# marcemq/crowdmod-ddpm-4D

Hardware: AMD Instinct MI355X
Metric: denoise-steps/sec (UNet fwd + sampler update) at ATC [B,4,T,H,W] (higher is better)
Workload: dtype f32; 1 GPU; config/ATC.yml sampling on the 12x36 grid, fp32 arithmetic (fp32 matrix instructions; fp32 products built from f16 two-way splits -- three v_mfma_f32_32x32x16_f16 cross terms, fp32 accumulate, same error against the reference as round 3's six-term bf16 form -- in the Winograd / quarter-resolution / last-conv layers, whose input is GroupNorm + SiLU output, and in the upsample layers, whose raw inpu; channels=4, past_len=5, future_len=3, global_batch=64, parallelism=batch-shard x1 (2 stream lanes of 32 chains per rank)

## Files before the change

### crowdmod-ddpm-4d_amd/csrc/cm_conv_wino.hip

```cpp
#include "cm_kernels.h"

#include <algorithm>
#include <atomic>
#include <map>
#include <mutex>
#include <tuple>
#include <vector>

namespace cm {

typedef float f32x16 __attribute__((ext_vector_type(16)));
typedef float f32x4 __attribute__((ext_vector_type(4)));
typedef _Float16 f16x8 __attribute__((ext_vector_type(8)));
typedef __bf16 bf16x8 __attribute__((ext_vector_type(8)));
typedef __bf16 bf16x4 __attribute__((ext_vector_type(4)));
typedef _Float16 f16x4 __attribute__((ext_vector_type(4)));

__device__ __forceinline__ float silu_w(float v) { return v * __builtin_amdgcn_rcpf(1.0f + __expf(-v)); }

typedef float f32x2 __attribute__((ext_vector_type(2)));
__device__ __forceinline__ f32x2 pk_sub2(f32x2 a, f32x2 b) {
  f32x2 r;
  asm("v_pk_add_f32 %0, %1, %2 neg_lo:[0,1] neg_hi:[0,1]" : "=v"(r) : "v"(a), "v"(b));
  return r;
// ... 390 lines not shown
  float *xb = XC + (size_t)(wave * 2) * 16 * 64 + lane;
#pragma unroll
  for (int reg = 0; reg < 16; ++reg) { xb[reg * 64] = t0[reg]; xb[(16 + reg) * 64] = t1[reg]; }
  __syncthreads();
  const int oa = wave >> 1, ob = wave & 1;
  f32x16 v;
  {
    const float *p0 = XC + (size_t)((0 * 2 + ob) * 16) * 64 + lane, *p1 = XC + (size_t)((1 * 2 + ob) * 16) * 64 + lane;
    const float *p2 = XC + (size_t)((2 * 2 + ob) * 16) * 64 + lane, *p3 = XC + (size_t)((3 * 2 + ob) * 16) * 64 + lane;
    if (oa == 0) {
#pragma unroll
      for (int reg = 0; reg < 16; ++reg) v[reg] = (p0[reg * 64] + p1[reg * 64]) + p2[reg * 64];
    } else {
#pragma unroll
      for (int reg = 0; reg < 16; ++reg) v[reg] = (p1[reg * 64] - p2[reg * 64]) - p3[reg * 64];
    }
  }
  if (n2 > 0) {
    for (int c0s = 0; c0s < n2; c0s += WINO_SKB) {
      if (c0s > 0) wino_skip_load(a, nt, n2a, n2, c0s, svox, lane, sa, sw);
      wino_skip_mfma(n2, c0s, sa, sw, v);
    }
  }
  wino_epilogue(a, v, outoff, nt, wave, lane, b0, bs, (((tz * a.nty + ty) * a.ntx) + tx) * 4 + wave, bias_pre, tv_pre);
}

#ifndef CM_WINO_ABL
#define CM_WINO_ABL 0
#endif
template <int BZ, int PY, int PX, bool F16, int NBW, bool SKIP, int B6 = 0, int FM = 0>
__global__ __launch_bounds__(256 * NBW, 2) void conv_wino_p_kernel(const ConvArgs a, const int *__restrict__ tabA,
                                                                  const int *__restrict__ tabO, int G) {
  constexpr bool ONE = (FM & WINO_FORM_ONE) != 0, PLAIN = (FM & WINO_FORM_PLAIN) != 0, OWNGN = (FM & WINO_FORM_OWNGN) != 0;
  constexpr bool WHOLE = (FM & WINO_FORM_WHOLE) != 0, AHEAD = (FM & WINO_FORM_AHEAD) != 0;
  static_assert(!AHEAD || (ONE && PLAIN && B6 == 3), "the halo-ahead order is a variant of the h2 one-sample forms");
  static_assert(!WHOLE || (BZ == 8 && PY == 2 && PX == 2 && NBW == 1), "the whole-tile form is the full-resolution tile's");
  static_assert(!OWNGN || PLAIN, "own GroupNorm is a variant of the plain activation form");
  constexpr int NT = 256 * NBW;
  constexpr int NP = PY * PX, ROWS = BZ * NP;
  static_assert(ROWS <= 32 && ROWS > 16, "one (partly filled) 32-row accumulator block per frequency component");
  constexpr int HZ = BZ + 2, UR = HZ * NP;
  static_assert(!(F16 && B6), "one operand format");
  constexpr bool SWZ = !F16 && !B6 && PY * PX == 4;
  constexpr bool CMP = B6 && BZ == 8;
  constexpr int URC = CMP ? (HZ - 1) * NP : UR;
  constexpr int CS = 16, S = CMP ? 24 : (B6 ? 28 : (F16 ? 12 : (SWZ ? CS : CS + 4)));
  constexpr int RYH = 2 * PY + 2, RXH = 2 * PX + 2, RV = HZ * RYH * RXH, RS_ = CMP ? 20 : (BZ == 8 ? 24 : 20);
  constexpr int PLV = RYH * RXH, RVC = CMP ? BZ * PLV : RV, RV0 = CMP ? PLV : 0;
  constexpr int RK = ((CMP ? BZ * RYH * RXH : RV) * 4 + NT - 1) / NT;
  constexpr int NITEMS = HZ * NP * (CS / 4);
  static_assert(NITEMS <= 256, "one staging item per thread");
  constexpr int USZ = 16 * URC * S, XSZ = NBW * 4 * 2 * 16 * 64;
  constexpr int UX = USZ > XSZ ? USZ : XSZ;
  extern __shared__ __attribute__((aligned(16))) float lds[];
  int *outoff = reinterpret_cast<int *>(lds);
  float *U = lds + 128;
  float *R = U + UX;
  float *GNL = R + RVC * RS_;

  const int tid = threadIdx.x, lane = tid & 63;
  const int wv8 = __builtin_amdgcn_readfirstlane(tid >> 6);
  const int wave = wv8 & 3, nbw = wv8 >> 2;
  const int r = lane & 31, hh = lane >> 5;
  const int g0 = blockIdx.x, p = blockIdx.y;
  const int nt = blockIdx.z * NBW + nbw;
  if (!ONE && g0 >= a.B) return;
  const int nc_epi = (WHOLE || nt * 32 + r < a.Co) ? nt * 32 + r : 0;
  const float bias_pre = a.bias[nc_epi];
// ... 91 lines not shown
      allv = allv && v4[0] >= 0 && v4[1] >= 0 && v4[2] >= 0 && v4[3] >= 0;
    }
  }
  const bool wave_all = WHOLE || (__all(allv) && nt * 32 + 31 < a.Co);
  const int n = nt * 32 + r;
  const bool nok = WHOLE || n < a.Co;
  const int n2a = SKIP ? a.s2C0 >> 5 : 0, n2 = SKIP ? (a.s2C0 + a.s2C1) >> 5 : 0;
  const int slot = p * 4 + wave;

  const bool own_gn = PLAIN ? OWNGN : a.gp0 != nullptr;
  const bool norm = PLAIN || a.gn != nullptr || own_gn;
  int b = g0;
  do {
    const bool more_b = !ONE && b + G < a.B;
    const float tv_pre = a.temb ? a.temb[(size_t)a.tidx[b] * a.temb_stride + nc_epi] : 0.f;
    if (own_gn) {
      __syncthreads();
      cm_gn_rows_from_slots(a, b, (int)Vs, GNL, U, tid, NT);
      __syncthreads();
    }
    f32x16 acc[4];
#pragma unroll
    for (int x = 0; x < 4; ++x)
#pragma unroll
      for (int i = 0; i < 16; ++i) acc[x][i] = 0.f;

    if constexpr (AHEAD) {
#pragma unroll
      for (int k = 0; k < RK; ++k) asm volatile("" : "+v"(ald[0][k]));
      if constexpr (!OWNGN) asm volatile("" : "+v"(scn[0]), "+v"(shn[0]));
      if (nchunks > 1) issue(NSL - 1, b, 1);
      asm volatile("" ::: "memory");
    }
    const int npair = AHEAD ? (nchunks & ~1) : nchunks;
#pragma unroll
    for (int pass = 0; pass < NSL; ++pass)
    for (int ch0 = pass ? npair : 0; ch0 < (pass ? nchunks : npair); ch0 += NSL)
#pragma unroll
    for (int SL = 0; SL < NSL - pass; ++SL) {
      const int ch = ch0 + SL;
      f32x4 sc1 = scn[SL], sh1 = shn[SL];
      if (own_gn) {
        const int cb0 = (ch < n0 ? ch * CS : a.C0 + (ch - n0) * CS) + 4 * aq;
        sc1 = *reinterpret_cast<const f32x4 *>(GNL + cb0);
        sh1 = *reinterpret_cast<const f32x4 *>(GNL + Ctot + cb0);
      }
      f32x4 pm1 = {1.f, 1.f, 1.f, 1.f};
      if (!((CM_WINO_ABL & 32) && ch > 0)) {
      if constexpr (!PLAIN) {
        if (a.pm) pm1 = *reinterpret_cast<const f32x4 *>(a.pm + (size_t)b * a.pm_stride + (ch < n0 ? ch * CS : a.C0 + (ch - n0) * CS) + 4 * aq);
      }
      if (PLAIN || (norm && a.silu && !a.pm)) {
#pragma unroll
        for (int k = 0; k < RK; ++k) {
          const int v = (tid >> 2) + (NT / 4) * k + RV0;
          f32x4 w = ald[SL][k] * sc1 + sh1;
          w[0] = silu_w(w[0]); w[1] = silu_w(w[1]); w[2] = silu_w(w[2]); w[3] = silu_w(w[3]);
          if (!((aok >> k) & 1u)) w = f32x4{0.f, 0.f, 0.f, 0.f};
          if (v >= RV0 && v < RV0 + RVC) *reinterpret_cast<f32x4 *>(R + (v - RV0) * RS_ + 4 * aq) = w;
        }
      } else {
#pragma unroll
        for (int k = 0; k < RK; ++k) {
          const int v = (tid >> 2) + (NT / 4) * k + RV0;
          f32x4 w = ald[SL][k];
          if (norm) {
            w = w * sc1 + sh1;
            if (a.silu) { w[0] = silu_w(w[0]); w[1] = silu_w(w[1]); w[2] = silu_w(w[2]); w[3] = silu_w(w[3]); }
          }
          if (a.pm) w = w * pm1;
          if (!((aok >> k) & 1u)) w = f32x4{0.f, 0.f, 0.f, 0.f};
          if (v >= RV0 && v < RV0 + RVC) *reinterpret_cast<f32x4 *>(R + (v - RV0) * RS_ + 4 * aq) = w;
        }
      }
      }
      __syncthreads();
      if constexpr (CMP) {
        if (ch == 0)
          for (int i = tid; i < 16 * 2 * NP * 3; i += NT) {
            const int xi = i / (2 * NP * 3), rem = i - xi * (2 * NP * 3), hf2 = rem / (NP * 3), r4 = rem - hf2 * (NP * 3);
            *reinterpret_cast<f32x4 *>(U + (size_t)xi * URC * S + (size_t)hf2 * URC * 12 + 4 * r4) = f32x4{0.f, 0.f, 0.f, 0.f};
          }
      }
      if (stager && !((CM_WINO_ABL & 4) && ch > 0)) {
        f32x4 d[16];
#pragma unroll
        for (int i = 0; i < 4; ++i)
#pragma unroll
          for (int j = 0; j < 4; ++j) d[i * 4 + j] = *reinterpret_cast<const f32x4 *>(R + rbase + (i * RXH + j) * RS_);
        auto put = [&](int k, const f32x4 v) {
          if constexpr (B6) {
            constexpr int NTW = B6 >= 2 ? 2 : 3;
            cm_u32x2_t t3[3];
            if constexpr (B6 == 3) cm_split2_f16(v, t3);
            else cm_split3_bf16<NTW>(v, t3);
#pragma unroll
            for (int tm = 0; tm < NTW; ++tm) *reinterpret_cast<cm_u32x2_t *>(uw + (size_t)k * URC * S + TST * tm) = t3[tm];
          } else if constexpr (F16) {
            const f16x4 hv = {(_Float16)v[0], (_Float16)v[1], (_Float16)v[2], (_Float16)v[3]};
            *reinterpret_cast<f16x4 *>(uw + (size_t)k * URC * S) = hv;
          } else {
            *reinterpret_cast<f32x4 *>(uw + (size_t)k * URC * S) = v;
          }
        };
        if constexpr (HX2) {
          f32x4 c[4][2];
// ... 11 lines not shown
            put(0 * 4 + j, pk_sub(e0, e2)); put(1 * 4 + j, e1 + e2); put(2 * 4 + j, pk_sub(e2, e1)); put(3 * 4 + j, pk_sub(e1, e3));
          }
        } else {
#pragma unroll
          for (int i = 0; i < 4; ++i) {
            const f32x4 e0 = d[i * 4 + 0], e1 = d[i * 4 + 1], e2 = d[i * 4 + 2], e3 = d[i * 4 + 3];
            d[i * 4 + 0] = pk_sub(e0, e2); d[i * 4 + 1] = e1 + e2; d[i * 4 + 2] = pk_sub(e2, e1); d[i * 4 + 3] = pk_sub(e1, e3);
          }
#pragma unroll
          for (int j = 0; j < 4; ++j) {
            const f32x4 e0 = d[0 * 4 + j], e1 = d[1 * 4 + j], e2 = d[2 * 4 + j], e3 = d[3 * 4 + j];
            d[0 * 4 + j] = pk_sub(e0, e2); d[1 * 4 + j] = e1 + e2; d[2 * 4 + j] = pk_sub(e2, e1); d[3 * 4 + j] = pk_sub(e1, e3);
          }
#pragma unroll
          for (int k = 0; k < 16; ++k) put(k, d[k]);
        }
      }
      __syncthreads();
#if !(CM_WINO_ABL & 2)
      if constexpr (!AHEAD) {
        if (ch + 1 < nchunks) issue(0, b, ch + 1);
        else if (more_b) issue(0, b + G, 0);
      }
#endif
      auto aread = [&](int g, f32x4 (&af)[4]) {
        const int dz = F16 ? g : g >> 1, k8 = F16 ? 0 : g & 1;
        const int acol = SWZ ? 4 * ((2 * k8 + hh) ^ (((ar >> 2) + dz) & 3)) : 8 * k8;
#pragma unroll
        for (int x = 0; x < 4; ++x) af[x] = *reinterpret_cast<const f32x4 *>(arow + (size_t)x * URC * S + (size_t)dz * NP * S + acol);
      };
      if constexpr (B6) {
        const float *ab = arow;
        f32x4 af6[2][3];
#pragma unroll
        for (int tm = 0; tm < 3; ++tm) af6[0][tm] = *reinterpret_cast<const f32x4 *>(ab + rowoff[0] + TST * tm);
#pragma unroll
        for (int sx = 0; sx < 12; ++sx) {
          const int g = sx >> 2, x = sx & 3;
          (void)g; (void)x;
          if (sx + 1 < 12) {
            const int g1 = (sx + 1) >> 2, x1 = (sx + 1) & 3;
#pragma unroll
            for (int tm = 0; tm < 3; ++tm)
              af6[(sx + 1) & 1][tm] = *reinterpret_cast<const f32x4 *>(ab + (size_t)x1 * URC * S + rowoff[g1] + TST * tm);
          }
          constexpr int TA[6] = {0, 2, 1, 0, 1, 0}, TB[6] = {2, 0, 1, 1, 0, 0};
#pragma unroll
          for (int u = (B6 >= 2 ? 3 : 0); u < ((CM_WINO_ABL & 8) ? (B6 >= 2 ? 4 : 1) : 6); ++u) {
            if constexpr (B6 == 3)
              acc[x] = __builtin_amdgcn_mfma_f32_32x32x16_f16(__builtin_bit_cast(f16x8, af6[sx & 1][TA[u]]),
                                                              __builtin_bit_cast(f16x8, b6[sx % RD6][TB[u]]), acc[x], 0, 0, 0);
            else
              acc[x] = __builtin_amdgcn_mfma_f32_32x32x16_bf16(__builtin_bit_cast(bf16x8, af6[sx & 1][TA[u]]),
                                                               __builtin_bit_cast(bf16x8, b6[sx % RD6][TB[u]]), acc[x], 0, 0, 0);
          }
          {
            constexpr int CHS = 4 * NG * 4 * 3 * 64;
            const int sn = sx + RD6;
            const bool wraps = sn >= 12;
            const bool more = !wraps || ch + 1 < nchunks || more_b;
            const int cn = !wraps ? ch : (ch + 1 < nchunks ? ch + 1 : 0);
            const f32x4 *wn = wbase + (size_t)cn * CHS + (size_t)((wraps ? sn - 12 : sn) * 3) * 64;
#if !(CM_WINO_ABL & 1)
            if (more) {
#pragma unroll
              for (int tm = 0; tm < 3; ++tm) b6[sx % RD6][tm] = wn[tm * 64];
            }
#else
            (void)wn; (void)more;
#endif
          }
          asm volatile("" ::: "memory");
        }
#if !(CM_WINO_ABL & 2)
        if constexpr (AHEAD) {
          if (pass == 0 && ch + 2 < nchunks) issue(SL, b, ch + 2);
          asm volatile("" ::: "memory");
        }
#endif
      } else {
#pragma unroll
      for (int g = 0; g < NG; ++g) {
        {
          const bool more = g < NG - 1 || ch + 1 < nchunks || more_b;
          const int cn = g < NG - 1 ? ch : (ch + 1 < nchunks ? ch + 1 : 0);
          const f32x4 *wn = wbase + (size_t)cn * (4 * NG * 4 * 64) + (size_t)(g < NG - 1 ? g + 1 : 0) * (4 * 64);
          if (more) {
#pragma unroll
            for (int x = 0; x < 4; ++x) bq[(g + 1) % RS][x] = wn[x * 64];
          }
        }
        f32x4 af[4];
        aread(g, af);
        if constexpr (F16) {
#pragma unroll
          for (int x = 0; x < 4; ++x)
            acc[x] = __builtin_amdgcn_mfma_f32_32x32x16_f16(__builtin_bit_cast(f16x8, af[x]), __builtin_bit_cast(f16x8, bq[g % RS][x]), acc[x], 0, 0, 0);
        } else {
#pragma unroll
          for (int jj = 0; jj < 4; ++jj)
#pragma unroll
            for (int x = 0; x < 4; ++x)
              acc[x] = __builtin_amdgcn_mfma_f32_32x32x2f32(af[x][jj], bq[g % RS][x][jj], acc[x], 0, 0, 0);
// ... 337 lines not shown
bool conv_wino_b6_ok(int bz, int by, int bx, int Co, int Zo) {
  if (cm::diag_env("CM_NO_WINO_P") || !conv_wino_tile_ok(bz, by, bx)) return false;
  const int nbw = conv_wino_nbw(bz, Co);
  if (bz != 8) return nbw == 2 && conv_wino_p_lds(bz, by, bx, false, 2, true) <= 160 * 1024;
  return nbw == 1 && by == 4 && bx == 4 && Zo == 8 && 2 * conv_wino_p_lds(bz, by, bx, false, 1, true) <= 160 * 1024 && !cm::diag_env("CM_NO_WINO_B6_FULL");
}

static size_t wino_p_lds_launch(const ConvArgs &a, bool f16, int nbw, bool b6, bool own_gn) {
  return conv_wino_p_lds(a.bz, a.by, a.bx, f16, nbw, b6) + (own_gn ? (size_t)2 * (a.C0 + a.C1) * sizeof(float) : 0);
}

bool conv_wino_p_taken(const ConvArgs &a, bool f16, bool own_gn) {
  static const bool no_p = cm::diag_env("CM_NO_WINO_P") != nullptr, all_p = cm::diag_env("CM_WINO_P") != nullptr;
  const int nbw = conv_wino_nbw_run(a, f16);
  const bool b6 = a.f16 == 2 || a.f16 == 3 || a.f16 == 4;
  return !no_p && conv_wino_two_step(a.bz, a.by, a.bx, f16, nbw) && (nbw == 2 || all_p || b6) &&
         wino_p_lds_launch(a, f16, nbw, b6, own_gn) <= 160 * 1024;
}

int conv_wino_form(const ConvArgs &a, int G) {
  if (a.dbg != 0 || a.f16 != 4) return 0;
  if (G < a.B || a.pm || !a.silu) return 0;
  const bool own = a.gp0 != nullptr;
  if (own == (a.gn != nullptr)) return 0;
  if (a.bz == 8) {
    const bool whole = a.by == 4 && a.bx == 4 && a.Yo % 4 == 0 && a.Xo % 4 == 0 && a.Zo % 8 == 0 && a.Co % 32 == 0;
    if (own || !whole || conv_wino_nbw(a.bz, a.Co) != 1) return 0;
    return WINO_FORM_ONE | WINO_FORM_PLAIN | WINO_FORM_WHOLE;
  }
  if (conv_wino_nbw(a.bz, a.Co) != 2) return 0;
  return WINO_FORM_ONE | WINO_FORM_PLAIN | (own ? WINO_FORM_OWNGN : 0);
}

static std::atomic<long long> wino_form_launches[16], wino_ahead_launches;
void conv_wino_form_counts(long long counts[16], bool reset) {
  for (int i = 0; i < 16; ++i) counts[i] = reset ? wino_form_launches[i].exchange(0) : wino_form_launches[i].load();
}
long long conv_wino_ahead_count(bool reset) { return reset ? wino_ahead_launches.exchange(0) : wino_ahead_launches.load(); }

hipError_t launch_conv_wino(const ConvArgs &a_in, bool f16, hipStream_t st) {
  ConvArgs a = a_in;
  a.dbg = conv_dbg_flags();
  if (!conv_wino_ok(a)) return hipErrorInvalidValue;
  const int nbw = conv_wino_nbw_run(a, f16);
  const bool b6 = a.f16 == 2 || a.f16 == 3 || a.f16 == 4;
  const bool t3 = a.f16 == 3, h2 = a.f16 == 4;
  if (b6 && (f16 || !conv_wino_b6_ok(a.bz, a.by, a.bx, a.Co, a.Zo))) return hipErrorInvalidValue;
#define CM_WINO_ATTR(KERNEL)                                                                        \
    static bool attr_set[64] = {false};                                                             \
    int dev = 0;                                                                                    \
    (void)hipGetDevice(&dev);                                                                       \
    if (!attr_set[dev & 63]) {                                                                      \
      hipError_t e = hipFuncSetAttribute(reinterpret_cast<const void *>(KERNEL), hipFuncAttributeMaxDynamicSharedMemorySize, 160 * 1024); \
      if (e != hipSuccess) return e;                                                                \
      attr_set[dev & 63] = true;                                                                    \
    }
  if (conv_wino_p_taken(a, f16, a.gp0 != nullptr)) {
    const size_t ldsp = wino_p_lds_launch(a, f16, nbw, b6, a.gp0 != nullptr);
    const int ntp = a.ntz * a.nty * a.ntx, nz = (a.Co + 31) / 32 / nbw;
    const int per_cu = (nbw == 1 && 2 * ldsp <= 160 * 1024) ? 2 : 1;
    const int slots = wino_cu_count() * per_cu;
    static const int g_force = cm::diag_env("CM_WINO_G") ? atoi(cm::diag_env("CM_WINO_G")) : 0;
    const int G = g_force > 0 ? std::min(a.B, g_force) : (b6 && nbw == 1) ? a.B : std::max(1, std::min(a.B, slots / std::max(1, ntp * nz)));
    WinoTabs tb;
    hipError_t et = wino_tabs_get(a, 256 * nbw, &tb);
    if (et != hipSuccess) return et;
    const dim3 gridp((unsigned)G, (unsigned)ntp, (unsigned)nz);
    static const bool no_ahead = cm::diag_env("CM_NO_WINO_AHEAD") != nullptr;
    const int fm0 = nbw == conv_wino_nbw(a.bz, a.Co) ? conv_wino_form(a, G) : 0;
    const int fm = fm0 && !no_ahead ? fm0 | WINO_FORM_AHEAD : fm0;
    int fm_run = 0;
#define CM_WINO_PGO1(KERNEL, THREADS)                                                               \
  {                                                                                                 \
    CM_WINO_ATTR(KERNEL)                                                                            \
    wino_form_launches[fm_run & 15].fetch_add(1, std::memory_order_relaxed);                        \
    if (fm_run & WINO_FORM_AHEAD) wino_ahead_launches.fetch_add(1, std::memory_order_relaxed);      \
    hipLaunchKernelGGL(KERNEL, gridp, dim3(THREADS), ldsp, st, a, tb.tA, tb.tO, G);                 \
    return hipGetLastError();                                                                       \
  }
#define CM_WINO_PGO(Z, PY_, PX_, F, NB, THREADS)                                                    \
  {                                                                                                 \
    if (a.s2w) CM_WINO_PGO1((conv_wino_p_kernel<Z, PY_, PX_, F, NB, true>), THREADS)                \
    CM_WINO_PGO1((conv_wino_p_kernel<Z, PY_, PX_, F, NB, false>), THREADS)                          \
  }
#define CM_WINO_PGOFM(Z, PY_, PX_, NB, THREADS, FM_)                                                \
    if (h2 && fm == (FM_)) {                                                                        \
      fm_run = (FM_);                                                                               \
      if (a.s2w) CM_WINO_PGO1((conv_wino_p_kernel<Z, PY_, PX_, false, NB, true, 3, (FM_)>), THREADS) \
      CM_WINO_PGO1((conv_wino_p_kernel<Z, PY_, PX_, false, NB, false, 3, (FM_)>), THREADS)          \
    }
#define CM_WINO_PGO6N(Z, PY_, PX_, NB, THREADS)                                                     \
  {                                                                                                 \
    if (h2) {                                                                                       \
      if (a.s2w) CM_WINO_PGO1((conv_wino_p_kernel<Z, PY_, PX_, false, NB, true, 3>), THREADS)       \
      CM_WINO_PGO1((conv_wino_p_kernel<Z, PY_, PX_, false, NB, false, 3>), THREADS)                 \
    }                                                                                               \
    if (t3) {                                                                                       \
      if (a.s2w) CM_WINO_PGO1((conv_wino_p_kernel<Z, PY_, PX_, false, NB, true, 2>), THREADS)       \
      CM_WINO_PGO1((conv_wino_p_kernel<Z, PY_, PX_, false, NB, false, 2>), THREADS)                 \
    }                                                                                               \
    if (a.s2w) CM_WINO_PGO1((conv_wino_p_kernel<Z, PY_, PX_, false, NB, true, 1>), THREADS)         \
    CM_WINO_PGO1((conv_wino_p_kernel<Z, PY_, PX_, false, NB, false, 1>), THREADS)                   \
  }
#define CM_WINO_PGO61(Z, PY_, PX_, THREADS) CM_WINO_PGO6N(Z, PY_, PX_, 1, THREADS)
#define CM_WINO_PGO6(Z, PY_, PX_, THREADS) CM_WINO_PGO6N(Z, PY_, PX_, 2, THREADS)
#define X(z, py, px)                                                                                \
    if (a.bz == z && a.by == 2 * py && a.bx == 2 * px) {                                            \
      if constexpr (z != 8) {                                                                       \
        if (nbw == 2 && b6) {                                                                       \
          CM_WINO_PGOFM(z, py, px, 2, 512, WINO_FORM_ONE | WINO_FORM_PLAIN)                         \
          CM_WINO_PGOFM(z, py, px, 2, 512, WINO_FORM_ONE | WINO_FORM_PLAIN | WINO_FORM_OWNGN)       \
          CM_WINO_PGOFM(z, py, px, 2, 512, WINO_FORM_ONE | WINO_FORM_PLAIN | WINO_FORM_AHEAD)       \
          CM_WINO_PGOFM(z, py, px, 2, 512, WINO_FORM_ONE | WINO_FORM_PLAIN | WINO_FORM_OWNGN | WINO_FORM_AHEAD) \
          CM_WINO_PGO6(z, py, px, 512)                                                              \
        }                                                                                           \
        if (nbw == 2 && f16) CM_WINO_PGO(z, py, px, true, 2, 512)                                   \
        if (nbw == 2) CM_WINO_PGO(z, py, px, false, 2, 512)                                         \
      }                                                                                             \
      if (f16) CM_WINO_PGO(z, py, px, true, 1, 256)                                                 \
      if constexpr (z == 8 && py == 2 && px == 2) {                                                 \
        if (b6) {                                                                                   \
          CM_WINO_PGOFM(z, py, px, 1, 256, WINO_FORM_ONE | WINO_FORM_PLAIN | WINO_FORM_WHOLE)       \
          CM_WINO_PGOFM(z, py, px, 1, 256, WINO_FORM_ONE | WINO_FORM_PLAIN | WINO_FORM_WHOLE | WINO_FORM_AHEAD) \
          CM_WINO_PGO61(z, py, px, 256)                                                             \
        }                                                                                           \
        CM_WINO_PGO(z, py, px, false, 1, 256)                                                       \
      }                                                                                             \
    }
    CM_WINO_TILES(X)
#undef X
  }
  if (b6) return hipErrorInvalidValue;
  if (a.gp0) return hipErrorInvalidValue;
  const dim3 grid((unsigned)(a.B * a.ntz * a.nty * a.ntx), (unsigned)((a.Co + 31) / 32 / nbw));
  const size_t lds = conv_wino_lds(a.bz, a.by, a.bx, f16, nbw);
#define CM_WINO_GO(KERNEL, THREADS)                                                                 \
  {                                                                                                 \
    CM_WINO_ATTR(KERNEL)                                                                            \
    hipLaunchKernelGGL(KERNEL, grid, dim3(THREADS), lds, st, a);                                    \
    return hipGetLastError();                                                                       \
  }
#define X(z, py, px)                                                                                \
  if (a.bz == z && a.by == 2 * py && a.bx == 2 * px) {                                              \
    constexpr bool two = (z == 8 && py == 2 && px == 2);                                            \
    if constexpr (z != 8) {                                                                         \
      if (nbw == 2 && f16) CM_WINO_GO((conv_wino_kernel<z, py, px, 2, true, true, 2>), 512)         \
      if (nbw == 2) CM_WINO_GO((conv_wino_kernel<z, py, px, 2, false, true, 2>), 512)               \
    }                                                                                               \
    if (f16) CM_WINO_GO((conv_wino_kernel<z, py, px, 2, true, true, 1>), 256)                       \
    CM_WINO_GO((conv_wino_kernel<z, py, px, 2, false, two, 1>), 256)                                \
  }
  CM_WINO_TILES(X)
#undef X
  return hipErrorInvalidValue;
}

// ... 525 lines not shown
```

### crowdmod-ddpm-4d_amd/csrc/cm_kernels.h

```cpp
#pragma once
#include <hip/hip_runtime.h>
#include <stdint.h>
#include <stdlib.h>
#include <vector>

namespace cm {

inline const char *diag_env(const char *name) {
  static const bool on = [] { const char *d = getenv("CM_DIAG"); return d && d[0] == '1' && d[1] == 0; }();
  return on ? getenv(name) : nullptr;
}

#ifdef __HIPCC__
typedef float cm_f32x2_t __attribute__((ext_vector_type(2)));
typedef float cm_f32x4_t __attribute__((ext_vector_type(4)));
typedef __bf16 cm_bf16x2_t __attribute__((ext_vector_type(2)));
typedef unsigned cm_u32x2_t __attribute__((ext_vector_type(2)));
typedef _Float16 cm_f16x4_t __attribute__((ext_vector_type(4)));
__device__ __forceinline__ unsigned cm_cvt_pk_bf16(float a, float b) {
  const cm_f32x2_t v = {a, b};
  return __builtin_bit_cast(unsigned, __builtin_convertvector(v, cm_bf16x2_t));
}
template <int NT = 3>
__device__ __forceinline__ void cm_split3_bf16(cm_f32x4_t x, cm_u32x2_t (&t)[3]) {
// ... 156 lines not shown
bool conv_zsplit_variant(const ConvArgs &a, int MB, int NB);
bool conv_par_f16_variant(int MB, int NB, int bz, int by, int bx);

extern int conv_dbg_override;
int conv_dbg_flags();
size_t conv_lds_bytes(const ConvArgs &a, int MB, int NB);
void conv_build_tables(const ConvArgs &a, int MB, int *hvtab , int *mtab );
int conv_halo_voxels(const ConvArgs &a);
hipError_t launch_conv(const ConvArgs &a, int MB, int NB, hipStream_t st);
bool conv1x1_f16_ok(const ConvArgs &a, int NB);
hipError_t launch_conv1x1_f16(const ConvArgs &a, int NB, hipStream_t st);
bool conv_variant_exists(int MB, int NB);
bool conv_ups_pick(int Z, int Y, int X, int *tz, int *ty, int *tx, int *mbw, int *planes);
bool conv_ups_ok(const ConvArgs &a, int mbw, int planes, int nbp);
int conv_ups_slots(const ConvArgs &a, int mbw);
hipError_t launch_conv_ups(const ConvArgs &a, int mbw, int planes, int nbp, hipStream_t st);
hipError_t launch_ups_b6_repack(const float *wfrag, long long wpar_stride, float *w6, long long w6_stride, int Co, int Ci, int NBP, hipStream_t st);
bool conv_smalln_ok(const ConvArgs &a, int MB);
size_t conv_smalln_lds(const ConvArgs &a, int MB);
hipError_t launch_conv_smalln(const ConvArgs &a, int MB, const float *wsm, hipStream_t st);

bool conv_first_ok(const ConvArgs &a, int cin);
int conv_first_blocks(const ConvArgs &a);
size_t conv_first_lds(const ConvArgs &a, int cin);
hipError_t launch_conv_first(const ConvArgs &a, int cin, const float *wpk, hipStream_t st);

bool conv_wino_tile_ok(int bz, int by, int bx);
bool conv_wino_ok(const ConvArgs &a);
size_t conv_wino_lds(int bz, int by, int bx, bool f16, int nbw);
int conv_wino_nbw(int bz, int Co);
int conv_wino_nbw_run(const ConvArgs &a, bool f16);
bool conv_wino_two_step(int bz, int by, int bx, bool f16, int nbw);
bool conv_wino_p_taken(const ConvArgs &a, bool f16, bool own_gn);
enum { WINO_FORM_ONE = 1, WINO_FORM_PLAIN = 2, WINO_FORM_OWNGN = 4, WINO_FORM_WHOLE = 8, WINO_FORM_AHEAD = 16 };
int conv_wino_form(const ConvArgs &a, int G);
void conv_wino_form_counts(long long counts[16], bool reset);
long long conv_wino_ahead_count(bool reset);
hipError_t launch_conv_wino(const ConvArgs &a, bool f16, hipStream_t st);
bool conv_wino_b6_ok(int bz, int by, int bx, int Co, int Zo);
hipError_t launch_wino_b6_repack(const float *wwino, float *w6, long long n_floats, hipStream_t st);
hipError_t launch_wgrad_wino(const ConvArgs &a, const float *dy, int dy_cs, float *part, int G, int ncb, int nkb, hipStream_t st);
hipError_t launch_wgrad_wino_f16(const ConvArgs &a, const float *dy, int dy_cs, float *part, int G, int ncb, int nkb, hipStream_t st);
hipError_t launch_wgrad_wino_reduce(const float *part, int G, int ncb, int nkb, int Co, int Ci, float *dW, hipStream_t st);
bool conv_wino_pick(int Zo, int Yo, int Xo, int *bz, int *by, int *bx);

struct QrArgs {
  const float *src0, *src1;
  int C0, C1;
  const float *part0, *cnt0;
  int ns0;
  const float *part1, *cnt1;
  int ns1;
  const float *gamma, *beta;
  int groups;
  float eps;
  int silu;
  float *gn_out;
  const float *wq6;
  int three;
  float h2_oscale;
  const float *wq;
  const float *bias;
  const float *temb;
  int temb_stride;
  const long long *tidx;
  const float *resid;
  int res_cs;
  float *out;
  int out_cs, Co, B, Y, X;
  float *stat_part, *stat_cnt;
// ... 459 lines not shown
```

### crowdmod-ddpm-4d_amd/csrc/cm_model.cpp

```cpp
#include <hip/hip_runtime.h>

#include <algorithm>
#include <cmath>
#include <cstdarg>
#include <cstdio>
#include <cstring>
#include <map>
#include <memory>
#include <numeric>
#include <set>
#include <string>
#include <thread>
#include <vector>

#include "../../include/crowdmod_hip.h"
#include "cm_kernels.h"
#include "cm_pack.h"

using namespace cm_pack;

namespace {

thread_local std::string g_err;

// ... 2510 lines not shown
  }
  tmp.skip_if_fused = false;
  tmp.dbg_h2 = mode == 2;
  if (mode == 1) { tmp.d_wwino_b6 = nullptr; tmp.d_wqr_b6 = nullptr; tmp.d_wups_b6 = nullptr; }
  int src_slots = 0;
  if (mode == 2 && op.ups && op.in0->part) {
    const Act *t = op.in0;
    src_slots = t->nslice;
    CM_HIP(cm::launch_chan_stats(t->d, B, t->V(), t->C, src_slots, t->part, t->cnt, st));
  }
  FwdPlan plan;
  const int rc = plan_debug_conv(m, tmp, index, B, src_slots, st, &plan) || run_conv(m, tmp, plan, plan.ops[index], st, 0, 0);
  const hipError_t e = hipStreamSynchronize(st);
  if (rc) return 1;
  if (e != hipSuccess) return fail("debug conv launch failed: %s", hipGetErrorString(e));
  CM_HIP(hipMemcpy(h_out, op.out_act->d, (size_t)B * Vo * op.out_act->C * sizeof(float), hipMemcpyDeviceToHost));
  return 0;
}

int cm_debug_wino_form_counts(int64_t counts[16], int32_t reset) {
  if (!counts) return fail("bad argument");
  long long c[16];
  cm::conv_wino_form_counts(c, reset != 0);
  for (int i = 0; i < 16; ++i) counts[i] = (int64_t)c[i];
  return 0;
}

int cm_debug_wino_ahead_count(int64_t *launches, int32_t reset) {
  if (!launches) return fail("bad argument");
  *launches = (int64_t)cm::conv_wino_ahead_count(reset != 0);
  return 0;
}

int cm_debug_conv_stats(cm_model *m, int32_t index, int32_t B, float *h_part, float *h_cnt, int32_t *nslots, int32_t *C) {
  CM_NOT_DIT(m, "cm_debug_conv_stats");
  if (check_ready(m, B)) return 1;
  if (!nslots || !C || index < 0 || index >= (int)m->ops.size()) return fail("bad argument");
  const Op &op = m->ops[index];
  if (op.kind != OP_CONV || !op.stat_act || !op.stat_act->part) return fail("op %d writes no statistics", index);
  const Act *t = op.stat_act;
  const int ns = (size_t)index < m->plan.ops.size() ? m->plan.ops[index].ns_out : 0;
  *nslots = ns; *C = t->C;
  DevGuard g(m->device);
  CM_HIP(hipStreamSynchronize(m->stream));
  if (h_part) CM_HIP(hipMemcpy(h_part, t->part, (size_t)B * ns * t->C * 2 * sizeof(float), hipMemcpyDeviceToHost));
  if (h_cnt) CM_HIP(hipMemcpy(h_cnt, t->cnt, (size_t)B * ns * sizeof(float), hipMemcpyDeviceToHost));
  return 0;
}

int cm_debug_time_conv(cm_model *m, int32_t index, int32_t MB, int32_t bz, int32_t by, int32_t bx, int32_t B,
                       int32_t iters, float *us) {
  CM_NOT_DIT(m, "cm_debug_time_conv");
  if (check_ready(m, B)) return 1;
  if (!us || index < 0 || index >= (int)m->ops.size() || iters < 1) return fail("bad argument");
  const Op &own = m->ops[index];
  if (own.kind != OP_CONV || ((own.first_k || own.wino) && MB > 0)) return fail("op %d is not a tunable convolution", index);
  DevGuard g(m->device);
  hipStream_t st = m->stream;
  Op op = own; op.skip_if_fused = false;
  int rc = 0;
  if (MB > 0) {
    cm::ConvArgs &a = op.ca;
    const int osd = a.par ? 2 : 1;
    if (bz < 1 || by < 1 || bx < 1 || (bz * by * bx + 31) / 32 != MB || !cm::conv_variant_exists(MB, op.NB)) rc = fail("invalid geometry");
    if (!rc) {
      a.bs = 1; a.bz = bz; a.by = by; a.bx = bx;
// ... 123 lines not shown
```

### crowdmod-ddpm-4d_amd/native.py

```python
from __future__ import annotations

import ctypes as C
import importlib.util
import os
from typing import Optional

import numpy as np

_HERE = os.path.dirname(os.path.abspath(__file__))
LIB_PATH = os.environ.get("CM_LIB_PATH") or os.path.join(_HERE, "libcrowdmod_hip.so")
MAX_LEVELS = 8
ABI_VERSION = 3


class NativeError(RuntimeError):
    """A libcrowdmod_hip call returned non-zero (message from cm_last_error)."""


class cm_unet_config(C.Structure):
    _fields_ = [
        ("in_channels", C.c_int32), ("out_channels", C.c_int32), ("num_res_blocks", C.c_int32),
        ("base_channels", C.c_int32), ("n_levels", C.c_int32),
        ("channel_mult", C.c_int32 * MAX_LEVELS), ("apply_attention", C.c_int32 * MAX_LEVELS),
        ("time_multiple", C.c_int32), ("rows", C.c_int32), ("cols", C.c_int32),
# ... 77 lines not shown
    "cm_schedule_destroy": (C.c_int, [_P]),
    "cm_schedule_table": (C.c_int, [_P, C.c_int32, _P, C.c_int32]),
    "cm_q_sample": (C.c_int, [_P, _P, _P, _P, _P, C.c_int32, C.c_int64, _P]),
    "cm_ddpm_step": (C.c_int, [_P, _P, _P, C.c_int32, _P, C.c_uint64, C.c_int64, C.c_int32, C.c_int64, _P]),
    "cm_sample_loop": (C.c_int, [_P, _P, _P, _P, _P, C.POINTER(cm_sample_opts), _P, _P, C.c_int32, _P]),
    "cm_sample_loop_host": (C.c_int, [_P, _P, _P, _P, _P, C.POINTER(cm_sample_opts), _P, _P, C.c_int32]),
    "cm_sample_num_steps": (C.c_int, [_P, C.POINTER(cm_sample_opts), C.POINTER(C.c_int32)]),
    "cm_profile_enable": (C.c_int, [_P, C.c_int32]),
    "cm_profile_read": (C.c_int, [_P, _F, C.POINTER(C.c_int64)]),
    "cm_profile_read_union": (C.c_int, [_P, _F]),
    "cm_profile_report": (C.c_int, [_P, C.c_char_p, C.c_int64]),
    "cm_model_cost": (C.c_int, [_P, C.c_int32, C.POINTER(C.c_double), C.POINTER(C.c_double)]),
    "cm_model_class_flops": (C.c_int, [_P, C.c_int32, C.POINTER(C.c_double)]),
    "cm_model_exec_flops": (C.c_int, [_P, C.c_int32, C.POINTER(C.c_double)]),
    "cm_train_exec_flops": (C.c_int, [_P, C.c_int32, C.POINTER(C.c_double), C.POINTER(C.c_double)]),
    "cm_model_issue_flops": (C.c_int, [_P, C.c_int32, C.POINTER(C.c_double), C.POINTER(C.c_double)]),
    "cm_frame_metrics": (C.c_int, [C.c_int32, _P, _P, C.c_int32, C.c_int32, C.c_int32, C.c_int32, C.c_int32, _P, _P]),
    "cm_ssim_frames": (C.c_int, [C.c_int32, _P, _P, C.c_int32, C.c_int32, C.c_int32, C.c_int32, C.c_int32, _P, _P]),
    "cm_energy": (C.c_int, [C.c_int32, _P, C.c_int32, C.c_int32, C.c_int32, C.c_int32, C.c_int32, C.c_float, C.c_float, _P, _P]),
    "cm_motion_feature_vectors": (C.c_int, [C.c_int32, _P, C.c_int32, C.c_int32, C.c_int32, C.c_int32, C.c_int32, C.c_int32,
                                            C.c_int32, C.c_double, _P, _P]),
    "cm_motion_feature_tables": (C.c_int, [C.c_int32, _P, _P, C.c_int32, C.c_int32, C.c_int32, C.c_int32, C.c_int32, C.c_int32,
                                           C.c_int32, C.c_double, _P]),
    "cm_mass_preservation_grad": (C.c_int, [C.c_int32, _P, C.c_int32, C.c_int32, C.c_int32, C.c_int32, C.c_int32,
                                            C.c_float, C.c_float, C.c_float, _P, _P]),
    "cm_debug_conv_flags": (C.c_int, [C.c_int32]),
    "cm_debug_conv_count": (C.c_int, [_P, C.POINTER(C.c_int32)]),
    "cm_debug_conv_info": (C.c_int, [_P, C.c_int32, C.c_char_p, C.c_int64]),
    "cm_debug_bwd_plan": (C.c_int, [_P, C.c_char_p, C.c_int64, C.POINTER(C.c_int64)]),
    "cm_debug_conv_io": (C.c_int, [_P, C.c_int32, C.c_int32, _P, _P, _P, C.c_int32]),
    "cm_debug_conv_stats": (C.c_int, [_P, C.c_int32, C.c_int32, _P, _P, _P, _P]),
    "cm_debug_wino_form_counts": (C.c_int, [_P, C.c_int32]),
    "cm_debug_wino_ahead_count": (C.c_int, [_P, C.c_int32]),
    "cm_debug_time_conv": (C.c_int, [_P, C.c_int32, C.c_int32, C.c_int32, C.c_int32, C.c_int32, C.c_int32, C.c_int32,
                                     C.POINTER(C.c_float)]),
    "cm_train_init": (C.c_int, [_P, C.c_float, C.c_float, C.c_float, C.c_float, C.c_float, C.c_float]),
    "cm_train_set_lr": (C.c_int, [_P, C.c_float]),
    "cm_train_set_autocast": (C.c_int, [_P, C.c_int32, C.c_int32]),
    "cm_train_get_autocast": (C.c_int, [_P, _P, _P]),
    "cm_train_set_sample_base": (C.c_int, [_P, C.c_int64]),
    "cm_train_step": (C.c_int, [_P, _P, _P, _P, _P, _P, _P, C.c_uint64, C.POINTER(C.c_float), C.c_int32, C.c_int32, _P]),
    "cm_train_step_xt": (C.c_int, [_P, _P, _P, _P, _P, _P, C.c_uint64, C.POINTER(C.c_float), C.c_int32, C.c_int32, _P]),
    "cm_train_get_grad": (C.c_int, [_P, C.c_char_p, _P, C.c_int64]),
    "cm_train_sync": (C.c_int, [_P]),
    "cm_train_flat_grads": (C.c_int, [_P, C.POINTER(_P), C.POINTER(C.c_int64)]),
    "cm_train_apply": (C.c_int, [_P, _P]),
    "cm_train_get_opt_state": (C.c_int, [_P, C.c_char_p, C.c_int32, _P, C.c_int64]),
    "cm_train_set_opt_state": (C.c_int, [_P, C.c_char_p, C.c_int32, _P, C.c_int64]),
    "cm_train_opt_step": (C.c_int, [_P, C.POINTER(C.c_int32), C.c_int32]),
    "cm_dit_train_init": (C.c_int, [_P, C.c_float, C.c_float, C.c_float, C.c_float, C.c_float, C.c_float]),
    "cm_dit_train_set_lr": (C.c_int, [_P, C.c_float]),
    "cm_dit_train_set_sample_base": (C.c_int, [_P, C.c_int64]),
    "cm_dit_train_step_xt": (C.c_int, [_P, _P, _P, _P, _P, C.c_uint64, C.POINTER(C.c_float), C.c_int32, C.c_int32, _P]),
    "cm_dit_train_flat_grads": (C.c_int, [_P, C.POINTER(_P), C.POINTER(C.c_int64)]),
    "cm_dit_train_apply": (C.c_int, [_P, _P]),
    "cm_dit_train_get_grad": (C.c_int, [_P, C.c_char_p, _P, C.c_int64]),
    "cm_dit_train_get_opt_state": (C.c_int, [_P, C.c_char_p, C.c_int32, _P, C.c_int64]),
    "cm_dit_train_set_opt_state": (C.c_int, [_P, C.c_char_p, C.c_int32, _P, C.c_int64]),
    "cm_dit_train_opt_step": (C.c_int, [_P, C.POINTER(C.c_int32), C.c_int32]),
    "cm_dit_train_sync": (C.c_int, [_P]),
    "cm_dit_train_get_pred": (C.c_int, [_P, _P, C.c_int64]),
    "cm_dit4d_train_init": (C.c_int, [_P, C.c_float, C.c_float, C.c_float, C.c_float, C.c_float, C.c_float]),
    "cm_dit4d_train_set_lr": (C.c_int, [_P, C.c_float]),
    "cm_dit4d_train_set_sample_base": (C.c_int, [_P, C.c_int64]),
    "cm_dit4d_train_set_autocast": (C.c_int, [_P, C.c_int32, C.c_int32]),
    "cm_dit4d_train_get_autocast": (C.c_int, [_P, _P, _P]),
# ... 171 lines not shown
```

### include/crowdmod_hip.h

```cpp
#ifndef CROWDMOD_HIP_H
#define CROWDMOD_HIP_H

#include <stddef.h>
#include <stdint.h>

#ifdef __cplusplus
extern "C" {
#endif

#define CM_ABI_VERSION 3
#define CM_MAX_LEVELS 8

typedef struct cm_model cm_model;
typedef struct cm_schedule cm_schedule;

typedef struct cm_unet_config {
  int32_t in_channels;
  int32_t out_channels;
  int32_t num_res_blocks;
  int32_t base_channels;
  int32_t n_levels;
  int32_t channel_mult[CM_MAX_LEVELS];
  int32_t apply_attention[CM_MAX_LEVELS];
  int32_t time_multiple;
// ... 120 lines not shown
int cm_profile_enable(cm_model *m, int32_t on);
int cm_profile_read(cm_model *m, float ms[8], int64_t launches[8]);
int cm_profile_read_union(cm_model *m, float ms[8]);
int cm_profile_report(cm_model *m, char *buf, int64_t capacity);
int cm_model_cost(const cm_model *m, int32_t B, double *flops, double *bytes);
int cm_model_class_flops(const cm_model *m, int32_t B, double flops[8]);
int cm_model_exec_flops(const cm_model *m, int32_t B, double flops[8]);
int cm_train_exec_flops(const cm_model *m, int32_t B, double flops[8], double f16[8]);
int cm_model_issue_flops(const cm_model *m, int32_t B, double f32[8], double b16[8]);

int cm_frame_metrics(int32_t device, const float *d_pred, const float *d_gt, int32_t N, int32_t C, int32_t H,
                     int32_t W, int32_t F, double *h_out, float *h_minmax);

int cm_ssim_frames(int32_t device, const float *d_pred, const float *d_gt, int32_t N, int32_t C, int32_t H, int32_t W,
                   int32_t F, const double *h_range, double *h_out);
int cm_energy(int32_t device, const float *d_x, int32_t N, int32_t C, int32_t H, int32_t W, int32_t L, float delta_t,
              float delta_l, const float *h_factor, double *h_out);
int cm_motion_feature_vectors(int32_t device, const float *d_seq, int32_t N, int32_t C, int32_t H, int32_t W, int32_t F,
                              int32_t f, int32_t k, double gamma, double *h_mf2, double *h_mf1);
int cm_motion_feature_tables(int32_t device, const float *d_pred, const float *d_gt, int32_t N, int32_t C, int32_t H,
                             int32_t W, int32_t F, int32_t f, int32_t k, double gamma, double *h_out);

int cm_mass_preservation_grad(int32_t device, const float *d_x, int32_t B, int32_t C, int32_t H, int32_t W, int32_t L,
                              float delta_t, float delta_l, float eps, float *d_grad, void *stream);

int cm_debug_conv_flags(int32_t flags);
int cm_debug_conv_count(const cm_model *m, int32_t *count);
int cm_debug_conv_info(const cm_model *m, int32_t index, char *buf, int64_t capacity);
int cm_debug_bwd_plan(const cm_model *m, char *buf, int64_t capacity, int64_t *needed);
int cm_debug_conv_io(cm_model *m, int32_t index, int32_t mode, const float *h_in0, const float *h_in1, float *h_out, int32_t B);
int cm_debug_conv_stats(cm_model *m, int32_t index, int32_t B, float *h_part, float *h_cnt, int32_t *nslots, int32_t *C);
int cm_debug_wino_form_counts(int64_t counts[16], int32_t reset);
int cm_debug_wino_ahead_count(int64_t *launches, int32_t reset);
int cm_debug_time_conv(cm_model *m, int32_t index, int32_t MB, int32_t bz, int32_t by, int32_t bx,
                       int32_t B, int32_t iters, float *us);

int cm_train_init(cm_model *m, float lr, float beta1, float beta2, float eps, float weight_decay,
                  float dropout_rate );
int cm_train_set_lr(cm_model *m, float lr);
int cm_train_set_autocast(cm_model *m, int32_t mode, int32_t loss_scale_log2);
int cm_train_get_autocast(const cm_model *m, int32_t *mode, int32_t *loss_scale_log2);
int cm_train_set_sample_base(cm_model *m, int64_t sample_id_base);
int cm_train_step(cm_model *m, const cm_schedule *s, const float *d_future, const float *d_past,
                  const int64_t *d_t, const float *d_eps, const float *d_dropmask, uint64_t seed,
                  float *h_loss, int32_t B, int32_t apply_update, void *stream);
int cm_train_flat_grads(cm_model *m, void **d_grads, int64_t *numel);
int cm_train_apply(cm_model *m, void *stream);
int cm_train_get_opt_state(cm_model *m, const char *name, int32_t which, float *h_out, int64_t numel);
int cm_train_set_opt_state(cm_model *m, const char *name, int32_t which, const float *h_in, int64_t numel);
int cm_train_opt_step(cm_model *m, int32_t *step, int32_t set);
int cm_train_step_xt(cm_model *m, const float *d_xt, const float *d_past, const int64_t *d_t,
                     const float *d_target, const float *d_dropmask, uint64_t seed, float *h_loss,
                     int32_t B, int32_t apply_update, void *stream);
int cm_train_get_grad(cm_model *m, const char *name, float *h_out, int64_t numel);
int cm_train_sync(cm_model *m);

int cm_dit_train_init(cm_model *m, float lr, float beta1, float beta2, float eps, float weight_decay,
                      float dropout_rate);
int cm_dit_train_set_lr(cm_model *m, float lr);
int cm_dit_train_set_sample_base(cm_model *m, int64_t sample_id_base);
int cm_dit_train_step_xt(cm_model *m, const float *d_xt, const float *d_past, const int64_t *d_t,
                         const float *d_target, uint64_t seed, float *h_loss, int32_t B, int32_t apply_update,
                         void *stream);
int cm_dit_train_flat_grads(cm_model *m, void **d_grads, int64_t *numel);
int cm_dit_train_apply(cm_model *m, void *stream);
int cm_dit_train_get_grad(cm_model *m, const char *name, float *h_out, int64_t numel);
// ... 81 lines not shown
```

Baseline: 979.3 denoise-steps/s, aggregate over 1 GPU under weak scaling (every GPU advances its own batch of 64 chains per step).

## Stage next chunk's GroupNorm+SiLU halo rounds inside the Winograd matrix phase

```diff
diff --git a/crowdmod-ddpm-4d_amd/csrc/cm_conv_wino.hip b/crowdmod-ddpm-4d_amd/csrc/cm_conv_wino.hip
--- a/crowdmod-ddpm-4d_amd/csrc/cm_conv_wino.hip
+++ b/crowdmod-ddpm-4d_amd/csrc/cm_conv_wino.hip
@@ -446,8 +446,9 @@
 __global__ __launch_bounds__(256 * NBW, 2) void conv_wino_p_kernel(const ConvArgs a, const int *__restrict__ tabA,
                                                                   const int *__restrict__ tabO, int G) {
   constexpr bool ONE = (FM & WINO_FORM_ONE) != 0, PLAIN = (FM & WINO_FORM_PLAIN) != 0, OWNGN = (FM & WINO_FORM_OWNGN) != 0;
-  constexpr bool WHOLE = (FM & WINO_FORM_WHOLE) != 0, AHEAD = (FM & WINO_FORM_AHEAD) != 0;
+  constexpr bool WHOLE = (FM & WINO_FORM_WHOLE) != 0, AHEAD = (FM & WINO_FORM_AHEAD) != 0, UNDER = (FM & WINO_FORM_UNDER) != 0;
   static_assert(!AHEAD || (ONE && PLAIN && B6 == 3), "the halo-ahead order is a variant of the h2 one-sample forms");
+  static_assert(!UNDER || AHEAD, "staging under the matrix phase reads the other slot of the halo-ahead buffer");
   static_assert(!WHOLE || (BZ == 8 && PY == 2 && PX == 2 && NBW == 1), "the whole-tile form is the full-resolution tile's");
   static_assert(!OWNGN || PLAIN, "own GroupNorm is a variant of the plain activation form");
   constexpr int NT = 256 * NBW;
@@ -605,6 +606,27 @@
       if (nchunks > 1) issue(NSL - 1, b, 1);
       asm volatile("" ::: "memory");
     }
+    auto gn_rows = [&](const int SLc, int chn, f32x4 &sc1, f32x4 &sh1) {
+      sc1 = scn[SLc]; sh1 = shn[SLc];
+      if (own_gn) {
+        const int cb0 = (chn < n0 ? chn * CS : a.C0 + (chn - n0) * CS) + 4 * aq;
+        sc1 = *reinterpret_cast<const f32x4 *>(GNL + cb0);
+        sh1 = *reinterpret_cast<const f32x4 *>(GNL + Ctot + cb0);
+      }
+    };
+    auto stage_round = [&](const int SLc, const int k, const f32x4 sc1, const f32x4 sh1) {
+      const int v = (tid >> 2) + (NT / 4) * k + RV0;
+      f32x4 w = ald[SLc][k] * sc1 + sh1;
+      w[0] = silu_w(w[0]); w[1] = silu_w(w[1]); w[2] = silu_w(w[2]); w[3] = silu_w(w[3]);
+      if (!((aok >> k) & 1u)) w = f32x4{0.f, 0.f, 0.f, 0.f};
+      if (v >= RV0 && v < RV0 + RVC) *reinterpret_cast<f32x4 *>(R + (v - RV0) * RS_ + 4 * aq) = w;
+    };
+    if constexpr (UNDER) {
+      f32x4 sc1, sh1;
+      gn_rows(0, 0, sc1, sh1);
+#pragma unroll
+      for (int k = 0; k < RK; ++k) stage_round(0, k, sc1, sh1);
+    }
     const int npair = AHEAD ? (nchunks & ~1) : nchunks;
 #pragma unroll
     for (int pass = 0; pass < NSL; ++pass)
@@ -612,12 +634,9 @@
 #pragma unroll
     for (int SL = 0; SL < NSL - pass; ++SL) {
       const int ch = ch0 + SL;
-      f32x4 sc1 = scn[SL], sh1 = shn[SL];
-      if (own_gn) {
-        const int cb0 = (ch < n0 ? ch * CS : a.C0 + (ch - n0) * CS) + 4 * aq;
-        sc1 = *reinterpret_cast<const f32x4 *>(GNL + cb0);
-        sh1 = *reinterpret_cast<const f32x4 *>(GNL + Ctot + cb0);
-      }
+      if constexpr (!UNDER) {
+      f32x4 sc1, sh1;
+      gn_rows(SL, ch, sc1, sh1);
       f32x4 pm1 = {1.f, 1.f, 1.f, 1.f};
       if (!((CM_WINO_ABL & 32) && ch > 0)) {
       if constexpr (!PLAIN) {
@@ -625,13 +644,7 @@
       }
       if (PLAIN || (norm && a.silu && !a.pm)) {
 #pragma unroll
-        for (int k = 0; k < RK; ++k) {
-          const int v = (tid >> 2) + (NT / 4) * k + RV0;
-          f32x4 w = ald[SL][k] * sc1 + sh1;
-          w[0] = silu_w(w[0]); w[1] = silu_w(w[1]); w[2] = silu_w(w[2]); w[3] = silu_w(w[3]);
-          if (!((aok >> k) & 1u)) w = f32x4{0.f, 0.f, 0.f, 0.f};
-          if (v >= RV0 && v < RV0 + RVC) *reinterpret_cast<f32x4 *>(R + (v - RV0) * RS_ + 4 * aq) = w;
-        }
+        for (int k = 0; k < RK; ++k) stage_round(SL, k, sc1, sh1);
       } else {
 #pragma unroll
         for (int k = 0; k < RK; ++k) {
@@ -645,6 +658,7 @@
           if (!((aok >> k) & 1u)) w = f32x4{0.f, 0.f, 0.f, 0.f};
           if (v >= RV0 && v < RV0 + RVC) *reinterpret_cast<f32x4 *>(R + (v - RV0) * RS_ + 4 * aq) = w;
         }
+      }
       }
       }
       __syncthreads();
@@ -722,6 +736,13 @@
       if constexpr (B6) {
         const float *ab = arow;
         f32x4 af6[2][3];
+        constexpr int UF = 6;
+        static_assert(!UNDER || (UF >= RD6 && UF + RK <= 12), "the rounds follow the ring wait that retires the halo, inside the phase");
+        const bool stage = UNDER && !(CM_WINO_ABL & 32) && pass == 0 && (SL == 0 || ch + 1 < nchunks);
+        f32x4 scu = {1.f, 1.f, 1.f, 1.f}, shu = {0.f, 0.f, 0.f, 0.f};
+        if constexpr (UNDER && OWNGN) {
+          if (pass == 0) gn_rows((SL + 1) & 1, min(ch + 1, nchunks - 1), scu, shu);
+        }
 #pragma unroll
         for (int tm = 0; tm < 3; ++tm) af6[0][tm] = *reinterpret_cast<const f32x4 *>(ab + rowoff[0] + TST * tm);
 #pragma unroll
@@ -759,6 +780,17 @@
 #else
             (void)wn; (void)more;
 #endif
+          }
+          if constexpr (UNDER) {
+            if (sx >= UF && sx - UF < RK && stage) {
+              asm volatile("" : "+v"(ald[(SL + 1) & 1][sx - UF]));
+              if constexpr (OWNGN) {
+                stage_round((SL + 1) & 1, sx - UF, scu, shu);
+              } else {
+                asm volatile("" : "+v"(scn[(SL + 1) & 1]), "+v"(shn[(SL + 1) & 1]));
+                stage_round((SL + 1) & 1, sx - UF, scn[(SL + 1) & 1], shn[(SL + 1) & 1]);
+              }
+            }
           }
           asm volatile("" ::: "memory");
         }
@@ -1162,11 +1194,12 @@
   return WINO_FORM_ONE | WINO_FORM_PLAIN | (own ? WINO_FORM_OWNGN : 0);
 }
 
-static std::atomic<long long> wino_form_launches[16], wino_ahead_launches;
+static std::atomic<long long> wino_form_launches[16], wino_ahead_launches, wino_under_launches;
 void conv_wino_form_counts(long long counts[16], bool reset) {
   for (int i = 0; i < 16; ++i) counts[i] = reset ? wino_form_launches[i].exchange(0) : wino_form_launches[i].load();
 }
 long long conv_wino_ahead_count(bool reset) { return reset ? wino_ahead_launches.exchange(0) : wino_ahead_launches.load(); }
+long long conv_wino_under_count(bool reset) { return reset ? wino_under_launches.exchange(0) : wino_under_launches.load(); }
 
 hipError_t launch_conv_wino(const ConvArgs &a_in, bool f16, hipStream_t st) {
   ConvArgs a = a_in;
@@ -1198,13 +1231,16 @@
     const dim3 gridp((unsigned)G, (unsigned)ntp, (unsigned)nz);
     static const bool no_ahead = cm::diag_env("CM_NO_WINO_AHEAD") != nullptr;
     const int fm0 = nbw == conv_wino_nbw(a.bz, a.Co) ? conv_wino_form(a, G) : 0;
-    const int fm = fm0 && !no_ahead ? fm0 | WINO_FORM_AHEAD : fm0;
+    static const bool no_under = cm::diag_env("CM_NO_WINO_UNDER") != nullptr;
+    const int fm1 = fm0 && !no_ahead ? fm0 | WINO_FORM_AHEAD : fm0;
+    const int fm = (fm1 & WINO_FORM_AHEAD) && !no_under && !(a.bz == 8 && a.s2w) ? fm1 | WINO_FORM_UNDER : fm1;
     int fm_run = 0;
 #define CM_WINO_PGO1(KERNEL, THREADS)                                                               \
   {                                                                                                 \
     CM_WINO_ATTR(KERNEL)                                                                            \
     wino_form_launches[fm_run & 15].fetch_add(1, std::memory_order_relaxed);                        \
     if (fm_run & WINO_FORM_AHEAD) wino_ahead_launches.fetch_add(1, std::memory_order_relaxed);      \
+    if (fm_run & WINO_FORM_UNDER) wino_under_launches.fetch_add(1, std::memory_order_relaxed);      \
     hipLaunchKernelGGL(KERNEL, gridp, dim3(THREADS), ldsp, st, a, tb.tA, tb.tO, G);                 \
     return hipGetLastError();                                                                       \
   }
@@ -1217,6 +1253,11 @@
     if (h2 && fm == (FM_)) {                                                                        \
       fm_run = (FM_);                                                                               \
       if (a.s2w) CM_WINO_PGO1((conv_wino_p_kernel<Z, PY_, PX_, false, NB, true, 3, (FM_)>), THREADS) \
+      CM_WINO_PGO1((conv_wino_p_kernel<Z, PY_, PX_, false, NB, false, 3, (FM_)>), THREADS)          \
+    }
+#define CM_WINO_PGOFM0(Z, PY_, PX_, NB, THREADS, FM_)     \
+    if (h2 && fm == (FM_) && !a.s2w) {                                                              \
+      fm_run = (FM_);                                                                               \
       CM_WINO_PGO1((conv_wino_p_kernel<Z, PY_, PX_, false, NB, false, 3, (FM_)>), THREADS)          \
     }
 #define CM_WINO_PGO6N(Z, PY_, PX_, NB, THREADS)                                                     \
@@ -1242,6 +1283,8 @@
           CM_WINO_PGOFM(z, py, px, 2, 512, WINO_FORM_ONE | WINO_FORM_PLAIN | WINO_FORM_OWNGN)       \
           CM_WINO_PGOFM(z, py, px, 2, 512, WINO_FORM_ONE | WINO_FORM_PLAIN | WINO_FORM_AHEAD)       \
           CM_WINO_PGOFM(z, py, px, 2, 512, WINO_FORM_ONE | WINO_FORM_PLAIN | WINO_FORM_OWNGN | WINO_FORM_AHEAD) \
+          CM_WINO_PGOFM(z, py, px, 2, 512, WINO_FORM_ONE | WINO_FORM_PLAIN | WINO_FORM_AHEAD | WINO_FORM_UNDER) \
+          CM_WINO_PGOFM(z, py, px, 2, 512, WINO_FORM_ONE | WINO_FORM_PLAIN | WINO_FORM_OWNGN | WINO_FORM_AHEAD | WINO_FORM_UNDER) \
           CM_WINO_PGO6(z, py, px, 512)                                                              \
         }                                                                                           \
         if (nbw == 2 && f16) CM_WINO_PGO(z, py, px, true, 2, 512)                                   \
@@ -1252,6 +1295,7 @@
         if (b6) {                                                                                   \
           CM_WINO_PGOFM(z, py, px, 1, 256, WINO_FORM_ONE | WINO_FORM_PLAIN | WINO_FORM_WHOLE)       \
           CM_WINO_PGOFM(z, py, px, 1, 256, WINO_FORM_ONE | WINO_FORM_PLAIN | WINO_FORM_WHOLE | WINO_FORM_AHEAD) \
+          CM_WINO_PGOFM0(z, py, px, 1, 256, WINO_FORM_ONE | WINO_FORM_PLAIN | WINO_FORM_WHOLE | WINO_FORM_AHEAD | WINO_FORM_UNDER) \
           CM_WINO_PGO61(z, py, px, 256)                                                             \
         }                                                                                           \
         CM_WINO_PGO(z, py, px, false, 1, 256)                                                       \
diff --git a/crowdmod-ddpm-4d_amd/csrc/cm_kernels.h b/crowdmod-ddpm-4d_amd/csrc/cm_kernels.h
--- a/crowdmod-ddpm-4d_amd/csrc/cm_kernels.h
+++ b/crowdmod-ddpm-4d_amd/csrc/cm_kernels.h
@@ -212,10 +212,11 @@
 int conv_wino_nbw_run(const ConvArgs &a, bool f16);
 bool conv_wino_two_step(int bz, int by, int bx, bool f16, int nbw);
 bool conv_wino_p_taken(const ConvArgs &a, bool f16, bool own_gn);
-enum { WINO_FORM_ONE = 1, WINO_FORM_PLAIN = 2, WINO_FORM_OWNGN = 4, WINO_FORM_WHOLE = 8, WINO_FORM_AHEAD = 16 };
+enum { WINO_FORM_ONE = 1, WINO_FORM_PLAIN = 2, WINO_FORM_OWNGN = 4, WINO_FORM_WHOLE = 8, WINO_FORM_AHEAD = 16, WINO_FORM_UNDER = 32 };
 int conv_wino_form(const ConvArgs &a, int G);
 void conv_wino_form_counts(long long counts[16], bool reset);
 long long conv_wino_ahead_count(bool reset);
+long long conv_wino_under_count(bool reset);
 hipError_t launch_conv_wino(const ConvArgs &a, bool f16, hipStream_t st);
 bool conv_wino_b6_ok(int bz, int by, int bx, int Co, int Zo);
 hipError_t launch_wino_b6_repack(const float *wwino, float *w6, long long n_floats, hipStream_t st);
diff --git a/crowdmod-ddpm-4d_amd/csrc/cm_model.cpp b/crowdmod-ddpm-4d_amd/csrc/cm_model.cpp
--- a/crowdmod-ddpm-4d_amd/csrc/cm_model.cpp
+++ b/crowdmod-ddpm-4d_amd/csrc/cm_model.cpp
@@ -2566,6 +2566,12 @@
   return 0;
 }
 
+int cm_debug_wino_under_count(int64_t *launches, int32_t reset) {
+  if (!launches) return fail("bad argument");
+  *launches = (int64_t)cm::conv_wino_under_count(reset != 0);
+  return 0;
+}
+
 int cm_debug_conv_stats(cm_model *m, int32_t index, int32_t B, float *h_part, float *h_cnt, int32_t *nslots, int32_t *C) {
   CM_NOT_DIT(m, "cm_debug_conv_stats");
   if (check_ready(m, B)) return 1;
diff --git a/crowdmod-ddpm-4d_amd/native.py b/crowdmod-ddpm-4d_amd/native.py
--- a/crowdmod-ddpm-4d_amd/native.py
+++ b/crowdmod-ddpm-4d_amd/native.py
@@ -133,6 +133,7 @@
     "cm_debug_conv_stats": (C.c_int, [_P, C.c_int32, C.c_int32, _P, _P, _P, _P]),
     "cm_debug_wino_form_counts": (C.c_int, [_P, C.c_int32]),
     "cm_debug_wino_ahead_count": (C.c_int, [_P, C.c_int32]),
+    "cm_debug_wino_under_count": (C.c_int, [_P, C.c_int32]),
     "cm_debug_time_conv": (C.c_int, [_P, C.c_int32, C.c_int32, C.c_int32, C.c_int32, C.c_int32, C.c_int32, C.c_int32,
                                      C.POINTER(C.c_float)]),
     "cm_train_init": (C.c_int, [_P, C.c_float, C.c_float, C.c_float, C.c_float, C.c_float, C.c_float]),
diff --git a/include/crowdmod_hip.h b/include/crowdmod_hip.h
--- a/include/crowdmod_hip.h
+++ b/include/crowdmod_hip.h
@@ -176,6 +176,7 @@
 int cm_debug_conv_stats(cm_model *m, int32_t index, int32_t B, float *h_part, float *h_cnt, int32_t *nslots, int32_t *C);
 int cm_debug_wino_form_counts(int64_t counts[16], int32_t reset);
 int cm_debug_wino_ahead_count(int64_t *launches, int32_t reset);
+int cm_debug_wino_under_count(int64_t *launches, int32_t reset);
 int cm_debug_time_conv(cm_model *m, int32_t index, int32_t MB, int32_t bz, int32_t by, int32_t bx,
                        int32_t B, int32_t iters, float *us);
 
```

Result: faster. 998.2 denoise-steps/s, aggregate over 1 GPU under weak scaling (every GPU advances its own batch of 64 chains per step), median of 6 (+1.9%).
